# ishine/Prior-DiffuSE

Hardware: AMD Instinct MI355X
Metric: enhanced-audio sec/sec (RTF), 6-step fast sampling, B=32 (higher is better)
Workload: dtype f16x2; 1 GPU; B=32 x 4 s 16 kHz utterances per GPU, [B,2,401,161] spectrograms, GCRN prior + DiffUNet1 6-step sampling, STFT..ISTFT, seeded random weights; global_batch=32, frames=401, parallelism=batch-shard x1, graph=True, streams_per_gpu=1, batches_in_flight=3

## Files before the change

include/pdse.h:

```cpp
#ifndef PDSE_H
#define PDSE_H
#include <stdint.h>

#ifdef __cplusplus
extern "C" {
#endif

#define PDSE_ABI_VERSION 9

typedef void* pdse_stream_t;

enum pdse_act { PDSE_ACT_NONE = 0, PDSE_ACT_PRELU = 1, PDSE_ACT_ELU = 2, PDSE_ACT_SIGMOID = 3 };

enum pdse_epi {
  PDSE_EPI_LINEAR = 0,
  PDSE_EPI_GLU = 1,
  PDSE_EPI_BIGLU = 2
};

typedef struct pdse_src {
  const float* ptr;
  int64_t sb, sc, st, sf;
  int32_t C;
  int32_t act;
// ... 277 lines not shown
  int32_t split;
  const float* x;
  const float* wih;
  const float* bih;
} pdse_gru_desc;

typedef struct pdse_transpose_desc {
  const float* in;
  float* out;
  int32_t N, R, Cc, pad_;
} pdse_transpose_desc;

typedef struct pdse_crm_desc {
  const float* x;
  const float* o;
  const float* ri;
  float* out;
  float a1, b1, a2, b2, a3, b3;
  int32_t plane, B, mode, pad_;
} pdse_crm_desc;

typedef struct pdse_gcrnlast_desc {
  const float* in0;
  const float* in1;
  const float* w1;
  const float* w2;
  const float* fcT;
  const float* fcb;
  float* out;
  int64_t out_sb;
  float b1, b2, bn_scale, bn_shift;
  int32_t B, T;
  const float* fcp;
} pdse_gcrnlast_desc;

typedef struct pdse_tcm_desc {
  const float* x;
  const float* h;
  float* x_out;
  float* h_out;
  const float* wbr;
  const float* bmain;
  const float* bmask;
  const float* xf;
  const float* wc2;
  const float* bc2;
  const float* xf2;
  const float* wn1;
  const float* bn1;
  float slope_main, slope_mask, slope2;
  int32_t dil, B, T;
  const int32_t* frames;
} pdse_tcm_desc;

typedef struct pdse_tcm2_desc {
  const float* x;
  float* x_out;
  const uint16_t* hs;
  uint16_t* hs_out;
  const uint16_t* wbr;
  const uint16_t* wc2;
  const uint16_t* wn1;
  const float* par;
  float slope2, slope_main_next, slope_mask_next;
  int32_t dil, B, T, mode;
  int32_t np;
// ... 269 lines not shown
```

prior-diffuse_amd/_lib.py:

```python
import contextlib
import ctypes as C
import os

_HERE = os.path.dirname(os.path.abspath(__file__))
LIB_PATH = os.environ.get("PDSE_LIB") or os.path.join(_HERE, "libpdse.so")

ABI_VERSION = 9

ACT_NONE, ACT_PRELU, ACT_ELU, ACT_SIGMOID = 0, 1, 2, 3
EPI_LINEAR, EPI_GLU, EPI_BIGLU = 0, 1, 2
EW_DIV, EW_UPDATE, EW_UPDATE_FINAL, EW_COPY, EW_ADD_MUL = 0, 1, 2, 3, 4
(OP_GCONV, OP_TIME, OP_EW, OP_COMPAND, OP_WAVPREP, OP_OLA, OP_SIGMA, OP_LN, OP_LSTM,
 OP_ROWLN, OP_CHLN, OP_ATTN, OP_GRU, OP_GNCOMB, OP_AHAM, OP_QSAMPLE, OP_TRANSPOSE, OP_TCM, OP_CRM, OP_GCRNLAST,
 OP_MASKLOSS, OP_GLSTM, OP_TCM2, OP_BGLU, OP_PLANES, OP_GLSTMP, OP_TCM2S, OP_DENSE, OP_ROWLNB, OP_METRICS, OP_RESAMPLE, OP_RANGE) = range(32)
MASKLOSS_BLOCKS = 32

_fp = C.c_void_p
_i32, _i64, _f32 = C.c_int32, C.c_int64, C.c_float


class Src(C.Structure):
    _fields_ = [("ptr", _fp), ("sb", _i64), ("sc", _i64), ("st", _i64), ("sf", _i64),
                ("C", _i32), ("act", _i32), ("blk", _i32), ("pad_", _i32)]

# ... 164 lines not shown
class BgluDesc(C.Structure):
    _fields_ = [("hp", _fp), ("hp_sb", _i64), ("hp_Tp", _i32), ("hp_Fp", _i32), ("hp_t0", _i32), ("hp_f0", _i32),
                ("x0", Src), ("x1", Src), ("Tin", _i32), ("Fin", _i32), ("ntaps", _i32), ("sf_in", _i32),
                ("tap_dt", _i32 * 10), ("tap_df", _i32 * 10), ("p1mask", _i32), ("Fout1", _i32),
                ("B", _i32), ("Tout", _i32), ("Fout", _i32), ("np", _i32),
                ("w0", _fp), ("w1", _fp), ("w2", _fp), ("w3", _fp), ("wlc", _fp), ("wrc", _fp), ("wc2", _fp), ("wc2v", _fp),
                ("nx_w", _fp), ("bias0", _fp), ("bias1", _fp), ("bias0_t0", _fp), ("bias1_t0", _fp), ("bias_sb", _i64),
                ("blc", _fp), ("brc", _fp), ("bc2", _fp), ("slope", _f32), ("C2", _i32),
                ("out", _fp), ("out_sb", _i64), ("out_sc", _i64), ("out_st", _i64), ("out_sf", _i64), ("out_off", _i64),
                ("hp_par", _i32), ("nx_n", _i32),
                ("nx_hp", _fp), ("nx_hp_sb", _i64), ("nx_Tp", _i32), ("nx_Fp", _i32), ("nx_t0", _i32), ("nx_f0", _i32),
                ("nx_row0", _i32), ("nx_par", _i32),
                ("nx_add", _fp), ("add_sb", _i64), ("add_sc", _i64), ("add_st", _i64), ("add_sf", _i64),
                ("nx_out", _fp * 2), ("nx_sb", _i64 * 2), ("nx_sc", _i64 * 2), ("nx_st", _i64 * 2), ("nx_sf", _i64 * 2),
                ("nx_bias", _fp * 3), ("nx_bias_sb", _i64 * 3), ("skip_Fh", _i32), ("nx_items", _i32), ("qexp", _i32 * 4)]


class PlanesDesc(C.Structure):
    _fields_ = [("in_", _fp), ("in_sb", _i64), ("in_sc", _i64), ("in_st", _i64), ("in_sf", _i64),
                ("hp", _fp), ("hp_sb", _i64), ("hp_Tp", _i32), ("hp_Fp", _i32), ("hp_t0", _i32), ("hp_f0", _i32),
                ("B", _i32), ("T", _i32), ("F", _i32), ("np", _i32),
                ("in1", _fp), ("w", _fp * 2), ("bias", _fp * 2), ("bias_sb", _i64), ("hp1", _fp),
                ("cin0", _i32), ("cin1", _i32), ("nd", _i32), ("pad_", _i32)]


class CrmDesc(C.Structure):
    _fields_ = [("x", _fp), ("o", _fp), ("ri", _fp), ("out", _fp), ("a1", _f32), ("b1", _f32), ("a2", _f32), ("b2", _f32),
                ("a3", _f32), ("b3", _f32), ("plane", _i32), ("B", _i32), ("mode", _i32), ("pad_", _i32)]


class GcrnLastDesc(C.Structure):
    _fields_ = [("in0", _fp), ("in1", _fp), ("w1", _fp), ("w2", _fp), ("fcT", _fp), ("fcb", _fp), ("out", _fp),
                ("out_sb", _i64), ("b1", _f32), ("b2", _f32), ("bn_scale", _f32), ("bn_shift", _f32), ("B", _i32), ("T", _i32),
                ("fcp", _fp)]


class MetricsDesc(C.Structure):
    _fields_ = [("clean", _fp), ("proc", _fp), ("lens_host", _fp), ("lens", _fp), ("tables", _fp), ("frames", _fp),
                ("sorted", _fp), ("out", _fp), ("B", _i32), ("Lmax", _i32), ("Mmax", _i32), ("measures", _i32),
                ("stoi_tables", _fp), ("stoi_work", _fp), ("stoi_out", _fp)]


class ResampleDesc(C.Structure):
    _fields_ = [("pcm", _fp), ("offs", _fp), ("n_in_host", _fp), ("n_in", _fp), ("taps", _fp), ("out", _fp),
                ("pcm_bytes", _i64), ("B", _i32), ("Lmax", _i32), ("up", _i32), ("down", _i32), ("half", _i32),
                ("width", _i32), ("ch", _i32), ("pad_", _i32)]


class RangeRow(C.Structure):
    _fields_ = [("ptr", _fp), ("n", _i64), ("s0", _i64), ("s1", _i64), ("s2", _i64),
                ("n0", _i32), ("n1", _i32), ("n2", _i32), ("n3", _i32), ("i0", _i32), ("par_half", _i32),
                ("kind", _i32), ("exp", _i32), ("out_row", _i32), ("pad_", _i32)]


class RangeDesc(C.Structure):
    _fields_ = [("rows", _fp), ("out", _fp),
                ("nrows", _i32), ("out_rows", _i32), ("mode", _i32), ("blocks", _i32)]


RANGE_BINS = 32
RANGE_F32, RANGE_F16HI = 0, 1
RANGE_CLEAR, RANGE_ACCUMULATE = 0, 1
RANGE_NONFINITE = 2
RANGE_BINADE = (None, float("-inf")) + tuple(range(-14, 15)) + (15,)
RANGE_BIN_FULL = RANGE_BINADE.index(-2)
RANGE_BIN_TOP = RANGE_BINS - 1

# ... 209 lines not shown
```

prior-diffuse_amd/csrc/capi.hip:

```cpp
#include <hip/hip_runtime.h>
#include <stdint.h>
#include <stdio.h>
#include <string.h>

#include <new>
#include <string>
#include <vector>

#include "pdse.h"
#include "pdse_internal.h"

static thread_local std::string g_err;

void pdse_set_error(const char* msg) { g_err = msg ? msg : "unknown error"; }

int pdse_check_hip(hipError_t e, const char* what) {
  if (e == hipSuccess) return 0;
  g_err = std::string(what) + ": " + hipGetErrorString(e);
  return 1;
}

int pdse_check_launch(const char* what) { return pdse_check_hip(hipGetLastError(), what); }

int pdse_lds_attr(const void* fn, unsigned long long* mask, const char* what) {
// ... 54 lines not shown
};

static int op_size(int kind) {
  switch (kind) {
#define X(KIND, stem, entry) case PDSE_OP_##KIND: return (int)sizeof(pdse_##stem##_desc);
    PDSE_OPS(X)
#undef X
    default: return -1;
  }
}

static int launch_op(const pdse_op& op, hipStream_t s) {
  switch (op.kind) {
#define X(KIND, stem, entry) case PDSE_OP_##KIND: return pdse_##stem##_launch(&op.d.stem, s);
    PDSE_OPS(X)
#undef X
    default: pdse_set_error("plan: unknown op kind"); return 1;
  }
}

static bool names_odd_phase(const pdse_op& op) {
  return op.kind == PDSE_OP_GCONV && op.d.gconv.korder == 5 && op.d.gconv.p1mask != 0 && op.d.gconv.w2 == nullptr;
}

static int check_follows(const pdse_plan* p, const pdse_op& op) {
  if (p->ops.empty() || !names_odd_phase(p->ops.back())) return 0;
  if (op.kind != PDSE_OP_GCONV) {
    pdse_set_error("plan: the operator behind a gconv that names its odd phase (p1mask, korder 5) must be that phase");
    return 1;
  }
  return pdse_gconv_pair_check(&p->ops.back().d.gconv, &op.d.gconv);
}

static int launch_at(const pdse_plan* p, const int i, const int end, hipStream_t s, int* n) {
  const pdse_op& op = p->ops[i];
  *n = 1;
  if (names_odd_phase(op) && i + 1 < end) {
    *n = 2;
    return pdse_gconv4_pair_launch(&op.d.gconv, &p->ops[i + 1].d.gconv, s);
  }
  return launch_op(op, s);
}

template <typename D>
static int validate_desc(const D*) { return 0; }
static int validate_desc(const pdse_range_desc* d) { return pdse_range_validate(d); }

extern "C" {

int pdse_abi_version(void) { return PDSE_ABI_VERSION; }
const char* pdse_last_error(void) { return g_err.c_str(); }
int pdse_desc_size(int op_kind) { return op_size(op_kind); }

#define X(KIND, stem, entry) \
  int entry(const pdse_##stem##_desc* d, pdse_stream_t s) { return validate_desc(d) ? 1 : pdse_##stem##_launch(d, (hipStream_t)s); }
PDSE_OPS(X)
#undef X

int pdse_plan_create(pdse_plan** out) {
  if (!out) {
    pdse_set_error("plan_create: null out");
    return 1;
  }
  *out = new (std::nothrow) pdse_plan();
  if (!*out) {
    pdse_set_error("plan_create: out of memory");
    return 1;
  }
  return 0;
// ... 384 lines not shown
```

prior-diffuse_amd/csrc/gconv4.hip:

```cpp
#include <hip/hip_runtime.h>
#include <stdint.h>
#include <stdio.h>
#include <stdlib.h>

#include "pdse.h"
#include "pdse_internal.h"

#include "gconv_common.h"

#ifndef G4_CH
#define G4_CH 3
#endif

__device__ __forceinline__ void glds16_g4(const void* g, void* l) {
  __builtin_amdgcn_global_load_lds((const __attribute__((address_space(1))) void*)g, (__attribute__((address_space(3))) void*)l,
                                   16, 0, 0);
}

__device__ __forceinline__ float g4_load(const float* sbase, const unsigned byte_off) {
  float v;
  asm volatile("global_load_dword %0, %1, %2" : "=v"(v) : "v"(byte_off), "s"(sbase) : "memory");
  return v;
}
typedef float g4_f32x4 __attribute__((ext_vector_type(4)));
// ... 29 lines not shown
__device__ __forceinline__ void g4_lds_read3(const unsigned addr, u32x4 (&a)[3]) {
  asm volatile("ds_read_b128 %0, %3\n\tds_read_b128 %1, %3 offset:1024\n\tds_read_b128 %2, %3 offset:2048"
               : "=&v"(a[0]), "=&v"(a[1]), "=&v"(a[2])
               : "v"(addr)
               : "memory");
}
__device__ __forceinline__ void g4_lds_read3(const unsigned addr, u32x4 (&a)[2]) {
  asm volatile("ds_read_b128 %0, %2\n\tds_read_b128 %1, %2 offset:1024" : "=&v"(a[0]), "=&v"(a[1]) : "v"(addr) : "memory");
}
__device__ __forceinline__ void g4_lds_read3(const unsigned addr, u32x4 (&a)[1]) {
  asm volatile("ds_read_b128 %0, %1" : "=&v"(a[0]) : "v"(addr) : "memory");
}
template <int N, int NP>
__device__ __forceinline__ void g4_lds_wait(u32x4 (&a)[N][NP]) {
  asm volatile("s_waitcnt lgkmcnt(0)" ::: "memory");
#pragma unroll
  for (int i = 0; i < N; ++i)
#pragma unroll
    for (int p = 0; p < NP; ++p) asm volatile("" : "+v"(a[i][p]));
}
__device__ __forceinline__ f32x16 g4_mfma6(const u32x4 (&a)[3], const uint4 (&b)[3], f32x16 acc) {
  const uint4 a1 = make_uint4(a[0][0], a[0][1], a[0][2], a[0][3]), a2 = make_uint4(a[1][0], a[1][1], a[1][2], a[1][3]),
              a3 = make_uint4(a[2][0], a[2][1], a[2][2], a[2][3]);
  acc = mfma_bf16(a1, b[2], acc);
  acc = mfma_bf16(a3, b[0], acc);
  acc = mfma_bf16(a2, b[1], acc);
  acc = mfma_bf16(a1, b[1], acc);
  acc = mfma_bf16(a2, b[0], acc);
  acc = mfma_bf16(a1, b[0], acc);
  return acc;
}
__device__ __forceinline__ f32x16 g4_mfma6(const u32x4 (&a)[2], const uint4 (&b)[2], f32x16 acc) {
  const uint4 a1 = make_uint4(a[0][0], a[0][1], a[0][2], a[0][3]), a2 = make_uint4(a[1][0], a[1][1], a[1][2], a[1][3]);
  acc = mfma_f16(a2, b[0], acc);
  acc = mfma_f16(a1, b[1], acc);
  acc = mfma_f16(a1, b[0], acc);
  return acc;
}
__device__ __forceinline__ f32x16 g4_mfma6(const u32x4 (&a)[1], const uint4 (&b)[1], f32x16 acc) {
  return mfma_bf16(make_uint4(a[0][0], a[0][1], a[0][2], a[0][3]), b[0], acc);
}
__device__ __forceinline__ uint32_t g4_pack_bf16(const float a, const float b) {
  typedef float f32x2 __attribute__((ext_vector_type(2)));
  typedef __bf16 bf16x2 __attribute__((ext_vector_type(2)));
  const f32x2 v = {a, b};
  union { bf16x2 h; uint32_t u; } c;
  c.h = __builtin_convertvector(v, bf16x2);
  return c.u;
}
__device__ __forceinline__ void g4_split(const float (&x)[8], uint4 (&b)[3]) { split8(x, b[0], b[1], b[2]); }
__device__ __forceinline__ void g4_split(const float (&x)[8], uint4 (&b)[2]) { split8h(x, pow2i(PDSE_F16_ACT_EXP), b[0], b[1]); }
__device__ __forceinline__ void g4_split(const float (&x)[8], uint4 (&b)[1]) {
  b[0] = make_uint4(g4_pack_bf16(x[0], x[1]), g4_pack_bf16(x[2], x[3]), g4_pack_bf16(x[4], x[5]), g4_pack_bf16(x[6], x[7]));
}

struct g4_chunk {
  int s, tap, cb0, n, kb0;
};

__device__ long long* g_trace4 = nullptr;

template <int EPI, int MT, bool BLK, int NP = 3>
__global__ __launch_bounds__(512, 2) void gconv4_kernel(const pdse_gconv_desc d) {
  constexpr int FB = 64 * NP;
#ifdef PDSE_DIAG
  long long* const trace = g_trace4;
#else
  long long* const trace = nullptr;
#endif
  const long long c_start = trace ? clock64() : 0;
// ... 571 lines not shown
```

prior-diffuse_amd/csrc/gconv_common.h:

```cpp
#ifndef PDSE_GCONV_COMMON_H
#define PDSE_GCONV_COMMON_H
#include <hip/hip_runtime.h>
#include <type_traits>
#include <stdint.h>

#include "pdse.h"

typedef float f32x16 __attribute__((ext_vector_type(16)));
typedef float f32x4 __attribute__((ext_vector_type(4)));

__device__ __forceinline__ int rho(int r, int h) { return (r & 3) + 8 * (r >> 2) + 4 * h; }

__device__ __forceinline__ float fast_exp(float x) { return __builtin_amdgcn_exp2f(x * 1.44269504088896340736f); }
__device__ __forceinline__ float sigmoid_f(float x) { return __builtin_amdgcn_rcpf(1.0f + fast_exp(-x)); }

template <int ACT>
__device__ __forceinline__ float act_c(float y, float slope) {
  if constexpr (ACT == PDSE_ACT_PRELU) return y > 0.f ? y : slope * y;
  else if constexpr (ACT == PDSE_ACT_ELU) return y > 0.f ? y : fast_exp(y) - 1.0f;
  else if constexpr (ACT == PDSE_ACT_SIGMOID) return sigmoid_f(y);
  else return y;
}

__device__ const float pdse_zeros[32] __attribute__((aligned(16))) = {0.f, 0.f, 0.f, 0.f, 0.f, 0.f, 0.f, 0.f, 0.f, 0.f, 0.f, 0.f, 0.f, 0.f, 0.f, 0.f,
// ... 61 lines not shown
}

__device__ __forceinline__ void split8(const float (&x)[8], uint4& p1, uint4& p2, uint4& p3) {
#ifdef PDSE_ABLATE_SPLIT
  p1 = make_uint4(__float_as_uint(x[0]), __float_as_uint(x[1]), __float_as_uint(x[2]), __float_as_uint(x[3]));
  p2 = make_uint4(__float_as_uint(x[4]), __float_as_uint(x[5]), __float_as_uint(x[6]), __float_as_uint(x[7]));
  p3 = make_uint4(p1.x ^ p2.x, p1.y ^ p2.y, p1.z ^ p2.z, p1.w ^ p2.w);
  return;
#endif
  uint32_t q1[4], q2[4], q3[4];
#pragma unroll
  for (int i = 0; i < 4; ++i) {
    const float a = x[2 * i], b = x[2 * i + 1];
    const float ra = a - __uint_as_float(__float_as_uint(a) & 0xffff0000u);
    const float rb = b - __uint_as_float(__float_as_uint(b) & 0xffff0000u);
    const float sa = ra - __uint_as_float(__float_as_uint(ra) & 0xffff0000u);
    const float sb = rb - __uint_as_float(__float_as_uint(rb) & 0xffff0000u);
    q1[i] = __builtin_amdgcn_perm(__float_as_uint(b), __float_as_uint(a), 0x07060302u);
    q2[i] = __builtin_amdgcn_perm(__float_as_uint(rb), __float_as_uint(ra), 0x07060302u);
    q3[i] = __builtin_amdgcn_perm(__float_as_uint(sb), __float_as_uint(sa), 0x07060302u);
  }
  p1 = make_uint4(q1[0], q1[1], q1[2], q1[3]);
  p2 = make_uint4(q2[0], q2[1], q2[2], q2[3]);
  p3 = make_uint4(q3[0], q3[1], q3[2], q3[3]);
}

typedef _Float16 f16x8 __attribute__((ext_vector_type(8)));

__device__ __forceinline__ f32x16 mfma_f16(const uint4& a, const uint4& b, const f32x16 c) {
  union { uint4 u; f16x8 v; } A, B;
  A.u = a;
  B.u = b;
  return __builtin_amdgcn_mfma_f32_32x32x16_f16(A.v, B.v, c, 0, 0, 0);
}

__device__ __forceinline__ float pow2i(const int e) { return __uint_as_float((uint32_t)(127 + e) << 23); }


__device__ __forceinline__ void split8h(const float (&x)[8], const float sc, uint4& p1, uint4& p2) {
  typedef float f32x2 __attribute__((ext_vector_type(2)));
  typedef _Float16 f16x2 __attribute__((ext_vector_type(2)));
  uint32_t q1[4], q2[4];
#pragma unroll
  for (int i = 0; i < 4; ++i) {
    const f32x2 t = {x[2 * i] * sc, x[2 * i + 1] * sc};
    union { f16x2 h; uint32_t u; } hi, lo;
    hi.h = __builtin_convertvector(t, f16x2);
    const f32x2 r = t - __builtin_convertvector(hi.h, f32x2);
    lo.h = __builtin_convertvector(r, f16x2);
    q1[i] = hi.u;
    q2[i] = lo.u;
  }
  p1 = make_uint4(q1[0], q1[1], q1[2], q1[3]);
  p2 = make_uint4(q2[0], q2[1], q2[2], q2[3]);
}

__device__ __forceinline__ f32x16 mfma6(const uint4* w, const uint4& b1, const uint4& b2, const uint4& b3, f32x16 acc) {
  const uint4 a1 = w[0], a2 = w[64], a3 = w[128];
  acc = mfma_bf16(a1, b3, acc);
  acc = mfma_bf16(a3, b1, acc);
  acc = mfma_bf16(a2, b2, acc);
  acc = mfma_bf16(a1, b2, acc);
  acc = mfma_bf16(a2, b1, acc);
  acc = mfma_bf16(a1, b1, acc);
  return acc;
}
// ... 545 lines not shown
```

prior-diffuse_amd/csrc/misc.hip:

```cpp
#include <hip/hip_runtime.h>
#include <stdint.h>

#include "pdse.h"
#include "pdse_internal.h"

#define REQ(cond, msg)          \
  do {                          \
    if (!(cond)) {              \
      pdse_set_error(msg);      \
      return 1;                 \
    }                           \
  } while (0)

__device__ __forceinline__ float silu_f(float x) { return x * (1.0f / (1.0f + expf(-x))); }

__global__ __launch_bounds__(1024) void time_embed_kernel(const pdse_time_desc d) {
  __shared__ float x0[128];
  __shared__ float y1[512];
  __shared__ float y2[512];
  const int b = blockIdx.x, j = threadIdx.x;
  const float t = d.t[b];
  if (j < 128) {
    float fl = floorf(t), ce = ceilf(t);
    int lo = (int)fl, hi = (int)ce;
    lo = min(max(lo, 0), d.max_steps - 1);
    hi = min(max(hi, 0), d.max_steps - 1);
    const float low = d.table[lo * 128 + j], high = d.table[hi * 128 + j];
    x0[j] = low + (high - low) * (t - fl);
  }
  __syncthreads();
  if (j < 512) {
    float s = d.b1[j];
    for (int i = 0; i < 128; ++i) s += d.p1T[i * 512 + j] * x0[i];
    y1[j] = silu_f(s);
  }
  __syncthreads();
  if (j < 512) {
// ... 313 lines not shown
    float t1, t2;
    if (d.mode == 0) {
      const float diff = d.label[off + i] - d.init[off + i];
      t1 = a * diff;
      t2 = s * d.noise[off + i];
    } else if (d.mode == 1) {
      t1 = a * d.label[off + i];
      const float ni = d.noise[off + i] + d.init[off + i];
      t2 = s * ni;
    } else {
      t1 = a * d.label[off + i];
      t2 = s * d.noise[off + i];
    }
    d.out[off + i] = t1 + t2;
  }
}

int pdse_qsample_launch(const pdse_qsample_desc* d, hipStream_t s) {
  REQ(d && d->label && d->noise && d->a && d->s && d->out, "qsample: null pointer");
  REQ(d->mode >= 0 && d->mode <= 2 && (d->mode == 2 || d->init), "qsample: mode 0 / 1 need init");
  REQ(d->B > 0 && d->B <= 65535 && d->plane > 0, "qsample: bad sizes");
  int bx = (int)((d->plane + 255) / 256);
  if (bx > 128) bx = 128;
  hipLaunchKernelGGL(qsample_kernel, dim3(bx, d->B), dim3(256), 0, s, *d);
  return pdse_check_launch("qsample");
}

#define GL_F 161
#define GL_FI 80
#define GL_KQ 21
#define GL_YB 132
__device__ __forceinline__ float gl_exp(float x) { return __builtin_amdgcn_exp2f(x * 1.44269504088896340736f); }

__global__ __launch_bounds__(512, 4) void gcrnlast_kernel(const pdse_gcrnlast_desc d) {
  typedef float f32x16 __attribute__((ext_vector_type(16)));
  __shared__ __attribute__((aligned(16))) float xs[2][2][32 * GL_FI];
  __shared__ __attribute__((aligned(16))) float ys[GL_KQ * 2 * GL_YB];
  __shared__ __attribute__((aligned(16))) float4 wl4[2][32];
  const int tid = threadIdx.x, lane = tid & 63, wave = tid >> 6;
  const int o = tid & 255, rr = tid >> 8;
  const bool act = o < GL_F;
  const bool odd = (o & 1) != 0;
  if (tid < 64) {
    const int c = tid & 31, par = tid >> 5;
    wl4[par][c] = par ? make_float4(d.w1[3 * c + 1], 0.f, d.w2[3 * c + 1], 0.f) : make_float4(d.w1[3 * c], d.w1[3 * c + 2], d.w2[3 * c], d.w2[3 * c + 2]);
  }
  for (int e = tid; e < GL_KQ * 2 * GL_YB; e += 512) ys[e] = 0.f;
  const int64_t plane = (int64_t)d.T * GL_FI;
  const int rows = d.B * d.T, ntiles = (rows + 31) >> 5;
  auto fetch = [&](const int row, float (&v)[10]) {
    const int rw = row < rows ? row : 0;
    const int b = rw / d.T, t = rw - b * d.T;
#pragma unroll
    for (int i = 0; i < 10; ++i) {
      const int e = o + 256 * i;
      const int c = e / GL_FI, f = e - c * GL_FI;
      v[i] = c < 16 ? d.in0[((int64_t)b * 16 + c) * plane + (int64_t)t * GL_FI + f]
                    : d.in1[((int64_t)b * 16 + (c - 16)) * plane + (int64_t)t * GL_FI + f];
    }
  };
  for (int tile = blockIdx.x; tile < ntiles; tile += gridDim.x) {
    const int row0 = tile * 32;
    float nxt[10];
    fetch(row0 + rr, nxt);
    __syncthreads();
    for (int it = 0; it < 16; ++it) {
      float* const xb = xs[it & 1][rr];
#pragma unroll
      for (int i = 0; i < 10; ++i) {
        const int e = o + 256 * i;
        const float v = nxt[i];
        xb[e] = e < 16 * GL_FI ? v : (v > 0.f ? v : gl_exp(v) - 1.0f);
      }
      if (it + 1 < 16) fetch(row0 + 2 * (it + 1) + rr, nxt);
      __syncthreads();
      if (act) {
        const int j = o >> 1;
        const bool has0 = odd || j < GL_FI, has2 = !odd && j >= 1;
        const int j0 = has0 ? j : GL_FI - 1, j2 = has2 ? j - 1 : 0;
        float m = 0.f, g = 0.f;
#pragma unroll 8
        for (int k = 0; k < 32; ++k) {
          const float4 w = wl4[odd ? 1 : 0][k];
          const float x0 = has0 ? xb[k * GL_FI + j0] : 0.f, x2 = has2 ? xb[k * GL_FI + j2] : 0.f;
          m += x0 * w.x + x2 * w.y;
          g += x0 * w.z + x2 * w.w;
        }
        float y = (m + d.b1) * __builtin_amdgcn_rcpf(1.0f + gl_exp(-(g + d.b2)));
        y = y * d.bn_scale + d.bn_shift;
        y = y > 0.f ? y : gl_exp(y) - 1.0f;
        ys[(2 * (o >> 3) + (o & 1)) * GL_YB + (2 * it + rr) * 4 + ((o >> 1) & 3)] = y;
      }
    }
    __syncthreads();
    if (wave < 6) {
      f32x16 acc;
#pragma unroll
      for (int r = 0; r < 16; ++r) acc[r] = 0.f;
      const float4* const B4 = reinterpret_cast<const float4*>(d.fcp) + (size_t)wave * GL_KQ * 64 + lane;
      const float* const A1 = ys + (lane >> 5) * GL_YB + (lane & 31) * 4;
#pragma unroll 7
      for (int kq = 0; kq < GL_KQ; ++kq) {
        const float4 bv = B4[(size_t)kq * 64];
        const float4 av = *reinterpret_cast<const float4*>(A1 + kq * 2 * GL_YB);
        acc = __builtin_amdgcn_mfma_f32_32x32x2f32(av.x, bv.x, acc, 0, 0, 0);
        acc = __builtin_amdgcn_mfma_f32_32x32x2f32(av.y, bv.y, acc, 0, 0, 0);
        acc = __builtin_amdgcn_mfma_f32_32x32x2f32(av.z, bv.z, acc, 0, 0, 0);
        acc = __builtin_amdgcn_mfma_f32_32x32x2f32(av.w, bv.w, acc, 0, 0, 0);
      }
      const int ob = 32 * wave + (lane & 31);
      if (ob < GL_F) {
        const float bias = d.fcb[ob];
#pragma unroll
        for (int r = 0; r < 16; ++r) {
          const int row = row0 + (r & 3) + 8 * (r >> 2) + 4 * (lane >> 5);
          if (row < rows) {
            const int b = row / d.T, t = row - b * d.T;
            d.out[(int64_t)b * d.out_sb + (int64_t)t * GL_F + ob] = acc[r] + bias;
          }
        }
      }
    }
  }
}

int pdse_gcrnlast_launch(const pdse_gcrnlast_desc* d, hipStream_t s) {
  REQ(d && d->in0 && d->in1 && d->w1 && d->w2 && d->fcT && d->fcp && d->fcb && d->out, "gcrn_last: null pointer");
  REQ(d->B > 0 && d->T > 0 && (int64_t)d->B * d->T < (1ll << 31), "gcrn_last: bad sizes");
  const int ntiles = (d->B * d->T + 31) / 32;
  hipLaunchKernelGGL(gcrnlast_kernel, dim3(ntiles < 512 ? ntiles : 512), dim3(512), 0, s, *d);
  return pdse_check_launch("gcrn_last");
}

__device__ __forceinline__ double block_sum_256(double v, double* lds) {
  for (int o = 32; o > 0; o >>= 1) v += __shfl_down(v, o);
  const int lane = threadIdx.x & 63, wave = threadIdx.x >> 6;
  if (lane == 0) lds[wave] = v;
  __syncthreads();
  double r = 0.0;
  if (threadIdx.x == 0) r = ((lds[0] + lds[1]) + lds[2]) + lds[3];
  return r;
}

__global__ __launch_bounds__(256) void maskloss_partial_kernel(const pdse_maskloss_desc d) {
  __shared__ double lds[4];
  const int b = blockIdx.y;
  const int fr = min(max(d.frames[b], 0), d.T);
  const int64_t plane = (int64_t)d.T * d.F, live = (int64_t)fr * d.F;
  double acc = 0.0;
  for (int c = 0; c < d.C; ++c) {
    const int64_t base = ((int64_t)b * d.C + c) * plane;
    for (int64_t i = (int64_t)blockIdx.x * 256 + threadIdx.x; i < live; i += (int64_t)gridDim.x * 256) {
      const float e = d.esti[base + i] - d.label[base + i];
      acc += (double)e * (double)e;
    }
  }
  const double tot = block_sum_256(acc, lds);
  if (threadIdx.x == 0) d.partial[(int64_t)b * gridDim.x + blockIdx.x] = tot;
}

__global__ __launch_bounds__(256) void maskloss_final_kernel(const pdse_maskloss_desc d) {
  __shared__ double lds[4];
  const int n = d.B * PDSE_MASKLOSS_BLOCKS;
// ... 18 lines not shown
```

prior-diffuse_amd/nets.py:

```python
import ctypes as C

import numpy as np
import torch

from . import _lib as L
from . import packing as P

F0 = 161
BIG = 1 << 30

TAG_NONE, TAG_EPS_BLOCK, TAG_EPS_CONV1, TAG_TCM, TAG_PRIOR, TAG_LSTM, TAG_SIGNAL, TAG_EW = range(8)


class WeightBank:

    def __init__(self):
        self.items = {}
        self.keep = []
        self.owners = []

    def token(self, obj):
        if obj is None:
            return None
        for i, o in enumerate(self.owners):
# ... 92 lines not shown
        self.descs.append((desc, tag))
        if self.plan is not None:
            self.plan.add(desc, tag)
        for op in self.f16x2_operands(desc):
            self._audit_ops.setdefault((op[0], op[1]), op)

    def named(self, name, t):
        self._audit_names[t.data_ptr()] = (name, t)
        return t

    @staticmethod
    def f16x2_operands(desc):
        out = []
        if isinstance(desc, L.BgluDesc) and desc.np == 2:
            if desc.hp:
                F_ = desc.hp_Fp - 2 * desc.hp_f0
                box = P.hp_box(desc.B, desc.hp_Tp - desc.hp_t0, F_, 2, par=bool(desc.hp_par))
                out.append((desc.hp + 2 * box["off"], L.RANGE_F16HI, box, ""))
            else:
                out += [(desc.x0.ptr, L.RANGE_F32, None, ""), (desc.x1.ptr, L.RANGE_F32, None, "")]
        elif isinstance(desc, L.Tcm2Desc) and desc.np == 2:
            out.append((desc.x, L.RANGE_F32, None, ""))
            if desc.mode == 0:
                for br, suffix in enumerate((".main", ".mask")):
                    box = P.tcm2_hs_box(desc.B, desc.T, 2, br)
                    out.append((desc.hs + 2 * box["off"], L.RANGE_F16HI, box, suffix))
        elif isinstance(desc, L.Tcm2sDesc):
            for i in range(desc.n):
                out += PlanBase.f16x2_operands(desc.blk[i])
        elif isinstance(desc, L.GconvDesc) and desc.korder == 5:
            out += [(s_.ptr, L.RANGE_F32, None, "") for s_ in (desc.in0, desc.in1) if s_.ptr]
        elif isinstance(desc, L.DenseDesc) and desc.np == 2:
            out.append((desc.D, L.RANGE_F32, None, ""))
        return [o for o in out if o[0]]

    def audited(self):
        out, seen = [], set()
        for addr, kind, box, suffix in self._audit_ops.values():
            hit = next(((n, t) for n, t in self._audit_names.values()
                        if t.data_ptr() <= addr < t.data_ptr() + t.numel() * t.element_size()), None)
            if hit is None:
                raise RuntimeError("range audit: the f16x2 operand at 0x%x lies in no buffer the builder named (PlanBase.named)" % addr)
            name, t = hit
            key = (name + suffix, kind)
            if key in seen:
                continue
            seen.add(key)
            out.append((name + suffix, t, kind, P.F16_ACT_EXP if kind == L.RANGE_F32 else 0,
                        None if box is None else dict(box, off=(addr - t.data_ptr()) // 2)))
        return out

    def finish(self):
        if self.plan is not None:
            self.plan.keep(self.ctx.keep, self.ctx.bank)

    def src(self, t, C_, sb, sc, st, sf, off=0, act=L.ACT_NONE, blk=0):
        return L.Src(Ctx.ptr(t, off), sb, sc, st, sf, C_, act, blk, 0)

    def gconv(self, *, in0, in1=None, Tin, Fin, taps, sf_in, W, Cout, bias0=None, bias0_sb=0,
              bias1=None, bias1_sb=0, epi=L.EPI_LINEAR, act=L.ACT_NONE, act_slope=0.0,
              padrow=None, padrow_sb=0, padrow_off=0, cin1=False, resid=None, out,
              out_strides, out_off=0, out_cr=1, B, Tout, Fout, tag=TAG_NONE, bias0_off=0, phase1=None, nx=None,
              bias1_off=0, bias_t0=None, label="gconv", s3=False, s3g=False, has_xf=False, flat=False):
        ctx = self.ctx
        d = L.GconvDesc()
        d.in0 = in0
# ... 695 lines not shown
                p = "%s.de%d.0" % (de, k)
                if k > 1:
                    o, ooff = self.dec[n & 1], 0
                    fn = lambda Fo: nchw_out(64, T, Fo)
                    bn, pr = "%s.de%d.2" % (de, k), "%s.de%d.3.weight" % (de, k)
                else:
                    o, ooff = out, di * T * F0
                    fn = lambda Fo: nchw_out(2, T, Fo)
                    bn, pr = None, None
                nx = None
                if chained and k > 1:
                    Fo = 2 * (Fin - 1) + 3
                    wn = lambda de=de, k=k: self.w("%s.de%d.0.conv1.weight" % (de, k - 1))[:, :, 0, 0].T[:, :64]
                    nx = dict(keep=False, row0=-1, tiles=[dict(wfn=wn, bias=self.zero32, out=Hn, add=self.Pskip[di][k - 1],
                                                                strides=(32 * T * Fo, T * Fo, Fo, 2))])
                Fin = self._biconvtransglu(step, 5 + 5 * di + n, p, k, in0, in1, Fin, o, fn, bn, pr, out_off=ooff, H=Hc,
                                           do_conv1=(k == 5 or not chained), nx=nx)
                if chained:
                    Hc, Hn = Hn, Hc
                in0 = self.src(o, 64, *nchw(64, T, Fin))
        return out


class GcrnPlan(PlanBase):
    fused_last = True
    fused_glstm = True
    split_bf16 = True
    gemm_planes = 2
    block8 = True
    fuse_phases = True
    flat_proj = True
    persist_lstm = True
    chunk_proj = True
    CHUNK_TC = 32
    PERSIST_MAX_B = 4
    ENC_C = [2, 16, 32, 64, 128, 256]
    ENC_F = [161, 80, 39, 19, 9, 4]

    def __init__(self, ctx, sd, B, T, plan=None, split_bf16=None, exclusive=False, planes=None):
        if split_bf16 is not None:
            self.split_bf16 = bool(split_bf16)
        if planes is not None:
            if planes not in (1, 2, 3) or (planes in (1, 2) and not self.split_bf16):
                raise ValueError("planes is 3 (bf16x3), 2 (f16x2) or 1 (bf16 mode); the one- and two-plane forms run on the GEMM kernels (split_bf16)")
            self.gemm_planes = int(planes)
        self.persist = bool(self.persist_lstm and self.fused_glstm and exclusive and B <= self.PERSIST_MAX_B and not self.force_generic)
        self.exclusive = bool(exclusive)
        self.chunk = bool(self.chunk_proj and self.fused_glstm and not exclusive and not self.persist and not self.force_generic
                          and T >= 2 * self.CHUNK_TC)
        super().__init__(ctx, plan, ns=(ctx.bank.token(sd), self.fused_last, self.fused_glstm, self.split_bf16, self.block8, self.persist,
                                        self.gemm_planes))
        self.sd, self.B, self.T = sd, B, T
        a = ctx.alloc
        self.Bp = Bp = (B + 31) // 32 * 32
        self.status = None
        self.x = a(B, 2, T, F0)
        self.out = a(B, 2, T, F0)
        self.e = [a(B, self.ENC_C[i + 1], T, self.ENC_F[i + 1]) for i in range(5)]
        self.gx = a(2, T, 2048, Bp, zero=True)
        R = 2 * self.CHUNK_TC if self.chunk else 2
        self.hT = a(R, 2, 512, Bp, zero=True)
        self.cst = a(2, 512, Bp, zero=True)
        self.y = a(B, T, 1024)
        if self.persist:
            bq = 1 << (B - 1).bit_length()
            self.gran = torch.zeros(4 * 1024 * bq, dtype=torch.int64, device=ctx.device)
            self.status = torch.zeros(4, dtype=torch.int32, device=ctx.device)
            ctx.keep += [self.gran, self.status]
        elif self.fused_glstm and not self.force_generic:
            self.hT2, self.cst2 = a(2, 2, 512, Bp, zero=True), a(2, 512, Bp, zero=True)
            self.gx2, self.part = a(R, 2, 2048, Bp, zero=True), a(R, 2, 64, Bp, 2, zero=True)
        else:
            self.yn = a(B, 1024, T)
        self.glstm = a(B, 256, T, 4)
        self.d = [a(B, 128, T, 9), a(B, 64, T, 19), a(B, 32, T, 39), a(B, 16, T, 80), a(B, 1, T, 161)]
        for i, t_ in enumerate(self.e):
            self.named("gcrn.e%d" % (i + 1), t_)
        self.named("gcrn.glstm", self.glstm)
        for i, t_ in enumerate(self.d[:4]):
            self.named("gcrn.d%d" % (5 - i), t_)
        self.named("gcrn.x", self.x)

# ... 109 lines not shown
            s = self.src(self.e[4], 128, *e_lay[4][0], off=128 * g * T * 4, blk=8 if blk else 0)
            return s, T, 4, [(0, f) for f in range(4)], wk, T, 1, 2048 * Bp, 0

        if self.persist:
            self._glstm_persistent(proj1)
        elif self.fused_glstm and not self.force_generic:
            self._glstm_wavefront(proj1)
        else:
            self._lstm_layer("lstm_list1", proj1, y_su=2, y_sg=1)
            self._ln("glstm.ln1", self.yn, 1024 * T, T, 0, 1, 1)

            def proj2(g):
                s = self.src(self.yn, 512, 1024 * T, T, 0, 1, off=512 * g * T)
                return s, 1, T, [(0, 0)], (lambda Wih: Wih.T), 1, T, 0, 2048 * Bp

            self._lstm_layer("lstm_list2", proj2, y_su=1, y_sg=512)
        if blk:
            self._ln("glstm.ln2", self.glstm, 256 * T * 4, T * 4 * 8, 8, 4 * 8, 4, blk=8)
        else:
            self._ln("glstm.ln2", self.glstm, 256 * T * 4, T * 4, 1, 4, 4)

        dec = [(5, 512, 128), (4, 256, 64), (3, 128, 32), (2, 64, 16), (1, 32, 1)]
        for br in (1, 2):
            in0 = self.src(self.glstm, 256, *(nc8(256, T, 4) if blk else nchw(256, T, 4)), blk=8 if blk else 0)
            in1 = self.src(self.e[4], 256, *e_lay[4][0], blk=8 if blk else 0)
            Fin = 4
            for n, (k, ci, co) in enumerate(dec):
                p = "conv%d_t_%d" % (k, br)
                Fout = 2 * (Fin - 1) + 3 + (1 if k == 2 else 0)
                if k == 1 and self.fused_last and not self.force_generic:
                    g = L.GcrnLastDesc()
                    self.apply(g, self.fields(p + ".last", lambda p=p, br=br: P.gcrn_last_fields(self.sd, p, br)))
                    g.in0, g.in1 = self.d[3].data_ptr(), self.e[0].data_ptr()
                    g.out, g.out_sb = Ctx.ptr(out, (br - 1) * T * F0), 2 * T * F0
                    g.B, g.T = B, T
                    self.add(g, TAG_PRIOR)
                    break
                dblk = blk and k >= 3
                fuse = self.fuse_phases and self.split_bf16 and self.gemm_planes == 2 and not self.force_generic
                ist, (osb, osc, olo, ost, osf), ocr = lay(dblk, co, Fout)
                for phase in (0, 1):
                    kk, taps = P.convT_phase_taps(1, 3, phase)
                    self.gconv(in0=in0, in1=in1, Tin=T, Fin=Fin, taps=taps, sf_in=1, Cout=co, epi=L.EPI_GLU, act=L.ACT_ELU,
                               W=lambda p=p, k=k, br=br, kk=kk: dict(
                                   wk0=P.convT_kmat(self.sd[p + ".conv1.weight"], kk),
                                   wk1=P.convT_kmat(self.sd[p + ".conv2.weight"], kk), bias0=self.w(p + ".conv1.bias"),
                                   bias1=self.w(p + ".conv2.bias"), post=P.bn_fold(self.sd, "bn%d_t_%d" % (k, br))),
                               out=self.d[n], out_strides=(osb, osc, olo, ost, 2 * osf), out_off=phase * osf, out_cr=ocr, B=B,
                               Tout=T, Fout=(Fout - phase + 1) // 2, tag=TAG_PRIOR, label="%s.ph%d" % (p, phase),
                               s3g=self.split_bf16, phase1=dict(mask=1, Fout1=Fout // 2) if phase == 0 and fuse and co <= 32 else None)
                Fin = Fout
                if k > 1:
                    in0 = self.src(self.d[n], co, *ist, blk=8 if dblk else 0)
                    skip = self.e[k - 2]
                    sblk = e_lay[k - 2][2] == 8
                    in1 = self.src(skip, co, *e_lay[k - 2][0], act=L.ACT_ELU, blk=8 if sblk else 0)
            else:
                self.gconv(in0=self.src(self.d[4], 1, *nchw(1, T, F0)), Tin=T, Fin=F0, taps=[(0, f) for f in range(F0)],
                           sf_in=1, W=lambda br=br: dict(wk0=self.w("fc%d.weight" % br).T, bias0=self.w("fc%d.bias" % br)),
                           Cout=F0, cin1=True, out=out, out_strides=(2 * T * F0, 1, 0, F0, 0), out_off=(br - 1) * T * F0, B=B,
                           Tout=T, Fout=1, tag=TAG_PRIOR, label="fc%d" % br)
        return out


class StftPlan(PlanBase):

    def __init__(self, ctx, B, L_, plan=None, normalize=True, split_bf16=False, reflect_own=False):
        super().__init__(ctx, plan, ns=("stft", bool(split_bf16)))
        self.split_bf16 = bool(split_bf16)
        if L_ <= 160:
            raise ValueError(f"utterance of {L_} samples: the centred STFT reflects 160 samples on each side (torch.stft "
                             "raises for the same input)")
        self.B, self.L = B, L_
        self.T = 1 + L_ // 160
        self.wav = ctx.alloc(B, L_)
        self.xpad = ctx.alloc(B, L_ + 320)
        self.c = ctx.alloc(B)
        self.lens = torch.full((B,), L_, dtype=torch.int32, device=ctx.device)
        ctx.keep.append(self.lens)
        self.feat = ctx.alloc(B, 2, self.T, F0)
        self.normalize = normalize
        self.reflect_own = bool(reflect_own)

# ... 424 lines not shown
```

Before: 10090 audio_s/s.

## Fuse last 16-channel transposed-conv stage into the GCRN final kernel

Adds a tail mode to the gcrn_last kernel that computes the preceding 16-channel transposed-conv GLU stage (both phases) per row tile with MFMA and writes its output straight into shared memory, instead of round-tripping through the d[3] buffer. The launcher detects the gconv pair followed by a matching gcrn_last op and launches only the fused kernel, skipping two gconv phase launches. This removes a global write/read of the intermediate activation and two launches. In exchange the fused kernel does more work per tile, uses only 5 waves for the tail compute, and adds barriers, which may hurt occupancy or overlap.

```diff
diff --git a/include/pdse.h b/include/pdse.h
--- a/include/pdse.h
+++ b/include/pdse.h
@@ -333,6 +333,19 @@
   float b1, b2, bn_scale, bn_shift;
   int32_t B, T;
   const float* fcp;
+  const float* t_in0;
+  const float* t_in1;
+  const float* t_w0e;
+  const float* t_w1e;
+  const float* t_w0o;
+  const float* t_w1o;
+  const float* t_bias0;
+  const float* t_bias1;
+  const float* t_post_scale;
+  const float* t_post_shift;
+  int64_t t_sb0, t_sc0, t_st0, t_sf0;
+  int64_t t_sb1, t_sc1, t_st1, t_sf1;
+  int32_t tail, t_wexp_e, t_wexp_o, pad_;
 } pdse_gcrnlast_desc;
 
 typedef struct pdse_tcm_desc {
diff --git a/prior-diffuse_amd/_lib.py b/prior-diffuse_amd/_lib.py
--- a/prior-diffuse_amd/_lib.py
+++ b/prior-diffuse_amd/_lib.py
@@ -220,7 +220,12 @@
 class GcrnLastDesc(C.Structure):
     _fields_ = [("in0", _fp), ("in1", _fp), ("w1", _fp), ("w2", _fp), ("fcT", _fp), ("fcb", _fp), ("out", _fp),
                 ("out_sb", _i64), ("b1", _f32), ("b2", _f32), ("bn_scale", _f32), ("bn_shift", _f32), ("B", _i32), ("T", _i32),
-                ("fcp", _fp)]
+                ("fcp", _fp),
+                ("t_in0", _fp), ("t_in1", _fp), ("t_w0e", _fp), ("t_w1e", _fp), ("t_w0o", _fp), ("t_w1o", _fp),
+                ("t_bias0", _fp), ("t_bias1", _fp), ("t_post_scale", _fp), ("t_post_shift", _fp),
+                ("t_sb0", _i64), ("t_sc0", _i64), ("t_st0", _i64), ("t_sf0", _i64),
+                ("t_sb1", _i64), ("t_sc1", _i64), ("t_st1", _i64), ("t_sf1", _i64),
+                ("tail", _i32), ("t_wexp_e", _i32), ("t_wexp_o", _i32), ("pad_", _i32)]
 
 
 class MetricsDesc(C.Structure):
diff --git a/prior-diffuse_amd/csrc/capi.hip b/prior-diffuse_amd/csrc/capi.hip
--- a/prior-diffuse_amd/csrc/capi.hip
+++ b/prior-diffuse_amd/csrc/capi.hip
@@ -110,9 +110,22 @@
   return pdse_gconv_pair_check(&p->ops.back().d.gconv, &op.d.gconv);
 }
 
+static bool absorbs_pair(const pdse_op& last, const pdse_op& d, const pdse_op& e) {
+  if (last.kind != PDSE_OP_GCRNLAST || e.kind != PDSE_OP_GCONV) return false;
+  const pdse_gcrnlast_desc& g = last.d.gcrnlast;
+  const pdse_gconv_desc &a = d.d.gconv, &b = e.d.gconv;
+  return g.tail == 1 && g.t_in0 == a.in0.ptr && g.t_in1 == a.in1.ptr && g.t_w0e == a.w0 && g.t_w1e == a.w1 && g.t_w0o == b.w0 &&
+         g.t_w1o == b.w1 && g.t_wexp_e == a.wexp && g.t_wexp_o == b.wexp && g.in0 == a.out && a.out == b.out && a.B == g.B &&
+         a.Tout == g.T;
+}
+
 static int launch_at(const pdse_plan* p, const int i, const int end, hipStream_t s, int* n) {
   const pdse_op& op = p->ops[i];
   *n = 1;
+  if (names_odd_phase(op) && i + 2 < end && absorbs_pair(p->ops[i + 2], op, p->ops[i + 1])) {
+    *n = 3;
+    return launch_op(p->ops[i + 2], s);
+  }
   if (names_odd_phase(op) && i + 1 < end) {
     *n = 2;
     return pdse_gconv4_pair_launch(&op.d.gconv, &p->ops[i + 1].d.gconv, s);
diff --git a/prior-diffuse_amd/csrc/gconv4.hip b/prior-diffuse_amd/csrc/gconv4.hip
--- a/prior-diffuse_amd/csrc/gconv4.hip
+++ b/prior-diffuse_amd/csrc/gconv4.hip
@@ -85,10 +85,7 @@
 }
 __device__ __forceinline__ f32x16 g4_mfma6(const u32x4 (&a)[2], const uint4 (&b)[2], f32x16 acc) {
   const uint4 a1 = make_uint4(a[0][0], a[0][1], a[0][2], a[0][3]), a2 = make_uint4(a[1][0], a[1][1], a[1][2], a[1][3]);
-  acc = mfma_f16(a2, b[0], acc);
-  acc = mfma_f16(a1, b[1], acc);
-  acc = mfma_f16(a1, b[0], acc);
-  return acc;
+  return mfma3_f16(a1, a2, b[0], b[1], acc);
 }
 __device__ __forceinline__ f32x16 g4_mfma6(const u32x4 (&a)[1], const uint4 (&b)[1], f32x16 acc) {
   return mfma_bf16(make_uint4(a[0][0], a[0][1], a[0][2], a[0][3]), b[0], acc);
diff --git a/prior-diffuse_amd/csrc/gconv_common.h b/prior-diffuse_amd/csrc/gconv_common.h
--- a/prior-diffuse_amd/csrc/gconv_common.h
+++ b/prior-diffuse_amd/csrc/gconv_common.h
@@ -117,6 +117,13 @@
   A.u = a;
   B.u = b;
   return __builtin_amdgcn_mfma_f32_32x32x16_f16(A.v, B.v, c, 0, 0, 0);
+}
+
+__device__ __forceinline__ f32x16 mfma3_f16(const uint4& a1, const uint4& a2, const uint4& b1, const uint4& b2, f32x16 acc) {
+  acc = mfma_f16(a2, b1, acc);
+  acc = mfma_f16(a1, b2, acc);
+  acc = mfma_f16(a1, b1, acc);
+  return acc;
 }
 
 __device__ __forceinline__ float pow2i(const int e) { return __uint_as_float((uint32_t)(127 + e) << 23); }
diff --git a/prior-diffuse_amd/csrc/misc.hip b/prior-diffuse_amd/csrc/misc.hip
--- a/prior-diffuse_amd/csrc/misc.hip
+++ b/prior-diffuse_amd/csrc/misc.hip
@@ -3,6 +3,8 @@
 
 #include "pdse.h"
 #include "pdse_internal.h"
+
+#include "gconv_common.h"
 
 #define REQ(cond, msg)          \
   do {                          \
@@ -382,8 +384,8 @@
 #define GL_YB 132
 __device__ __forceinline__ float gl_exp(float x) { return __builtin_amdgcn_exp2f(x * 1.44269504088896340736f); }
 
+template <bool TAIL>
 __global__ __launch_bounds__(512, 4) void gcrnlast_kernel(const pdse_gcrnlast_desc d) {
-  typedef float f32x16 __attribute__((ext_vector_type(16)));
   __shared__ __attribute__((aligned(16))) float xs[2][2][32 * GL_FI];
   __shared__ __attribute__((aligned(16))) float ys[GL_KQ * 2 * GL_YB];
   __shared__ __attribute__((aligned(16))) float4 wl4[2][32];
@@ -402,11 +404,78 @@
     const int rw = row < rows ? row : 0;
     const int b = rw / d.T, t = rw - b * d.T;
 #pragma unroll
-    for (int i = 0; i < 10; ++i) {
+    for (int i = TAIL ? 5 : 0; i < 10; ++i) {
       const int e = o + 256 * i;
       const int c = e / GL_FI, f = e - c * GL_FI;
       v[i] = c < 16 ? d.in0[((int64_t)b * 16 + c) * plane + (int64_t)t * GL_FI + f]
                     : d.in1[((int64_t)b * 16 + (c - 16)) * plane + (int64_t)t * GL_FI + f];
+    }
+  };
+  auto tail_rows = [&](const int first) {
+    const int n = 32 * wave + (lane & 31), hh = lane >> 5;
+    const int rl = n / 40, j = n - 40 * rl;
+    f32x16 ae, ao;
+    if (wave < 5) {
+      const int row = first + rl, rw = row < rows ? row : 0;
+      const int b = rw / d.T, t = rw - b * d.T;
+#pragma unroll
+      for (int r = 0; r < 16; ++r) ae[r] = ao[r] = 0.f;
+      const bool gate = (lane & 16) != 0;
+      const int wl = lane - (gate ? 16 : 0);
+      const uint4* const we = reinterpret_cast<const uint4*>(gate ? d.t_w1e : d.t_w0e) + wl;
+      const uint4* const wo = reinterpret_cast<const uint4*>(gate ? d.t_w1o : d.t_w0o) + wl;
+#pragma unroll 1
+      for (int s = 0; s < 2; ++s) {
+        const float* const sp = (s ? d.t_in1 : d.t_in0) + (int64_t)b * (s ? d.t_sb1 : d.t_sb0) + (int64_t)t * (s ? d.t_st1 : d.t_st0);
+        const int ssc = (int)(s ? d.t_sc1 : d.t_sc0), ssf = (int)(s ? d.t_sf1 : d.t_sf0);
+#pragma unroll
+        for (int tap = 0; tap < 2; ++tap) {
+          const int fin = j - tap;
+          const bool inb = fin >= 0 && fin < 39;
+#pragma unroll
+          for (int cb = 0; cb < 2; ++cb) {
+            const float* const q = sp + ((inb ? fin : 0) * ssf + (2 * cb + hh) * ssc);
+            const float4 v0 = *reinterpret_cast<const float4*>(q), v1 = *reinterpret_cast<const float4*>(q + 4);
+            float x[8] = {v0.x, v0.y, v0.z, v0.w, v1.x, v1.y, v1.z, v1.w};
+#pragma unroll
+            for (int e = 0; e < 8; ++e) x[e] = inb ? x[e] : 0.f;
+            if (s) {
+#pragma unroll
+              for (int e = 0; e < 8; ++e) x[e] = x[e] < 0.f ? fast_exp(x[e]) - 1.0f : x[e];
+            }
+            uint4 b1, b2;
+            split8h(x, pow2i(PDSE_F16_ACT_EXP), b1, b2);
+            const uint4* const fe = we + (size_t)((s * 2 + tap) * 2 + cb) * 128;
+            ae = mfma3_f16(fe[0], fe[64], b1, b2, ae);
+            if (tap == 0) {
+              const uint4* const fo = wo + (size_t)(s * 2 + cb) * 128;
+              ao = mfma3_f16(fo[0], fo[64], b1, b2, ao);
+            }
+          }
+        }
+      }
+      const float ue = pow2i(-(PDSE_F16_ACT_EXP + d.t_wexp_e)), uo = pow2i(-(PDSE_F16_ACT_EXP + d.t_wexp_o));
+#pragma unroll
+      for (int r = 0; r < 16; ++r) {
+        ae[r] *= ue;
+        ao[r] *= uo;
+      }
+    }
+    __syncthreads();
+    if (wave < 5) {
+      float* const xo = xs[rl >> 1][rl & 1] + 2 * j;
+      const float *pb0 = d.t_bias0 + 4 * hh, *pb1 = d.t_bias1 + 4 * hh, *ps = d.t_post_scale + 4 * hh, *pt = d.t_post_shift + 4 * hh;
+#pragma unroll
+      for (int r = 0; r < 8; ++r) {
+        float y = ae[r] + pb0[PDSE_KR(r)];
+        y = y * sigmoid_f(ae[r + 8] + pb1[PDSE_KR(r)]);
+        y = y * ps[PDSE_KR(r)] + pt[PDSE_KR(r)];
+        xo[(PDSE_KR(r) + 4 * hh) * GL_FI] = act_c<PDSE_ACT_ELU>(y, 0.f);
+        float z = ao[r] + pb0[PDSE_KR(r)];
+        z = z * sigmoid_f(ao[r + 8] + pb1[PDSE_KR(r)]);
+        z = z * ps[PDSE_KR(r)] + pt[PDSE_KR(r)];
+        xo[(PDSE_KR(r) + 4 * hh) * GL_FI + 1] = act_c<PDSE_ACT_ELU>(z, 0.f);
+      }
     }
   };
   for (int tile = blockIdx.x; tile < ntiles; tile += gridDim.x) {
@@ -415,9 +484,10 @@
     fetch(row0 + rr, nxt);
     __syncthreads();
     for (int it = 0; it < 16; ++it) {
+      if (TAIL && !(it & 1)) tail_rows(row0 + 2 * it);
       float* const xb = xs[it & 1][rr];
 #pragma unroll
-      for (int i = 0; i < 10; ++i) {
+      for (int i = TAIL ? 5 : 0; i < 10; ++i) {
         const int e = o + 256 * i;
         const float v = nxt[i];
         xb[e] = e < 16 * GL_FI ? v : (v > 0.f ? v : gl_exp(v) - 1.0f);
@@ -475,10 +545,25 @@
 }
 
 int pdse_gcrnlast_launch(const pdse_gcrnlast_desc* d, hipStream_t s) {
-  REQ(d && d->in0 && d->in1 && d->w1 && d->w2 && d->fcT && d->fcp && d->fcb && d->out, "gcrn_last: null pointer");
+  REQ(d && d->in1 && d->w1 && d->w2 && d->fcT && d->fcp && d->fcb && d->out, "gcrn_last: null pointer");
   REQ(d->B > 0 && d->T > 0 && (int64_t)d->B * d->T < (1ll << 31), "gcrn_last: bad sizes");
+  REQ(d->tail == 0 || d->tail == 1, "gcrn_last: tail is 0 or 1");
   const int ntiles = (d->B * d->T + 31) / 32;
-  hipLaunchKernelGGL(gcrnlast_kernel, dim3(ntiles < 512 ? ntiles : 512), dim3(512), 0, s, *d);
+  const dim3 grid(ntiles < 512 ? ntiles : 512);
+  if (d->tail) {
+    REQ(d->t_in0 && d->t_in1 && d->t_w0e && d->t_w1e && d->t_w0o && d->t_w1o && d->t_bias0 && d->t_bias1 && d->t_post_scale &&
+            d->t_post_shift,
+        "gcrn_last: tail = 1 needs the sources, packed weights, biases and folded BatchNorm of the 16-channel stage");
+    REQ(!((d->t_sb0 | d->t_sc0 | d->t_st0 | d->t_sf0 | d->t_sb1 | d->t_sc1 | d->t_st1 | d->t_sf1) & 3) &&
+            !((reinterpret_cast<uintptr_t>(d->t_in0) | reinterpret_cast<uintptr_t>(d->t_in1) | reinterpret_cast<uintptr_t>(d->t_w0e) |
+               reinterpret_cast<uintptr_t>(d->t_w1e) | reinterpret_cast<uintptr_t>(d->t_w0o) | reinterpret_cast<uintptr_t>(d->t_w1o)) & 15),
+        "gcrn_last: the tail's sources are channel-blocked (strides in multiples of 4 floats), sources and weights 16-byte aligned");
+    REQ(d->t_wexp_e >= -40 && d->t_wexp_e <= 40 && d->t_wexp_o >= -40 && d->t_wexp_o <= 40, "gcrn_last: tail weight exponent out of range");
+    hipLaunchKernelGGL(gcrnlast_kernel<true>, grid, dim3(512), 0, s, *d);
+    return pdse_check_launch("gcrn_last tail");
+  }
+  REQ(d->in0, "gcrn_last: null pointer");
+  hipLaunchKernelGGL(gcrnlast_kernel<false>, grid, dim3(512), 0, s, *d);
   return pdse_check_launch("gcrn_last");
 }
 
diff --git a/prior-diffuse_amd/nets.py b/prior-diffuse_amd/nets.py
--- a/prior-diffuse_amd/nets.py
+++ b/prior-diffuse_amd/nets.py
@@ -148,6 +148,8 @@
             out += [(s_.ptr, L.RANGE_F32, None, "") for s_ in (desc.in0, desc.in1) if s_.ptr]
         elif isinstance(desc, L.DenseDesc) and desc.np == 2:
             out.append((desc.D, L.RANGE_F32, None, ""))
+        elif isinstance(desc, L.GcrnLastDesc) and desc.tail:
+            out += [(desc.t_in0, L.RANGE_F32, None, ""), (desc.t_in1, L.RANGE_F32, None, "")]
         return [o for o in out if o[0]]
 
     def audited(self):
@@ -909,6 +911,8 @@
     flat_proj = True
     persist_lstm = True
     chunk_proj = True
+    fused_tail = True
+    TAIL_MIN_ROWS = 1024
     CHUNK_TC = 32
     PERSIST_MAX_B = 4
     ENC_C = [2, 16, 32, 64, 128, 256]
@@ -925,6 +929,8 @@
         self.exclusive = bool(exclusive)
         self.chunk = bool(self.chunk_proj and self.fused_glstm and not exclusive and not self.persist and not self.force_generic
                           and T >= 2 * self.CHUNK_TC)
+        self.tail = bool(self.fused_tail and B * T >= self.TAIL_MIN_ROWS and self.split_bf16 and self.gemm_planes == 2
+                         and self.fused_last and self.block8 and not self.force_generic)
         super().__init__(ctx, plan, ns=(ctx.bank.token(sd), self.fused_last, self.fused_glstm, self.split_bf16, self.block8, self.persist,
                                         self.gemm_planes))
         self.sd, self.B, self.T = sd, B, T
@@ -1100,6 +1106,14 @@
                     g = L.GcrnLastDesc()
                     self.apply(g, self.fields(p + ".last", lambda p=p, br=br: P.gcrn_last_fields(self.sd, p, br)))
                     g.in0, g.in1 = self.d[3].data_ptr(), self.e[0].data_ptr()
+                    if self.tail:
+                        pe, po = tail_ph
+                        g.tail, g.t_in0, g.t_in1 = 1, pe.in0.ptr, pe.in1.ptr
+                        g.t_sb0, g.t_sc0, g.t_st0, g.t_sf0 = pe.in0.sb, pe.in0.sc, pe.in0.st, pe.in0.sf
+                        g.t_sb1, g.t_sc1, g.t_st1, g.t_sf1 = pe.in1.sb, pe.in1.sc, pe.in1.st, pe.in1.sf
+                        g.t_w0e, g.t_w1e, g.t_w0o, g.t_w1o = pe.w0, pe.w1, po.w0, po.w1
+                        g.t_bias0, g.t_bias1, g.t_post_scale, g.t_post_shift = pe.bias0, pe.bias1, pe.post_scale, pe.post_shift
+                        g.t_wexp_e, g.t_wexp_o = pe.wexp, po.wexp
                     g.out, g.out_sb = Ctx.ptr(out, (br - 1) * T * F0), 2 * T * F0
                     g.B, g.T = B, T
                     self.add(g, TAG_PRIOR)
@@ -1107,16 +1121,19 @@
                 dblk = blk and k >= 3
                 fuse = self.fuse_phases and self.split_bf16 and self.gemm_planes == 2 and not self.force_generic
                 ist, (osb, osc, olo, ost, osf), ocr = lay(dblk, co, Fout)
+                tail_ph = []
                 for phase in (0, 1):
                     kk, taps = P.convT_phase_taps(1, 3, phase)
-                    self.gconv(in0=in0, in1=in1, Tin=T, Fin=Fin, taps=taps, sf_in=1, Cout=co, epi=L.EPI_GLU, act=L.ACT_ELU,
-                               W=lambda p=p, k=k, br=br, kk=kk: dict(
-                                   wk0=P.convT_kmat(self.sd[p + ".conv1.weight"], kk),
-                                   wk1=P.convT_kmat(self.sd[p + ".conv2.weight"], kk), bias0=self.w(p + ".conv1.bias"),
-                                   bias1=self.w(p + ".conv2.bias"), post=P.bn_fold(self.sd, "bn%d_t_%d" % (k, br))),
-                               out=self.d[n], out_strides=(osb, osc, olo, ost, 2 * osf), out_off=phase * osf, out_cr=ocr, B=B,
-                               Tout=T, Fout=(Fout - phase + 1) // 2, tag=TAG_PRIOR, label="%s.ph%d" % (p, phase),
-                               s3g=self.split_bf16, phase1=dict(mask=1, Fout1=Fout // 2) if phase == 0 and fuse and co <= 32 else None)
+                    tail_ph.append(self.gconv(
+                        in0=in0, in1=in1, Tin=T, Fin=Fin, taps=taps, sf_in=1, Cout=co,
+                        epi=L.EPI_GLU, act=L.ACT_ELU,
+                        W=lambda p=p, k=k, br=br, kk=kk: dict(
+                            wk0=P.convT_kmat(self.sd[p + ".conv1.weight"], kk),
+                            wk1=P.convT_kmat(self.sd[p + ".conv2.weight"], kk), bias0=self.w(p + ".conv1.bias"),
+                            bias1=self.w(p + ".conv2.bias"), post=P.bn_fold(self.sd, "bn%d_t_%d" % (k, br))),
+                        out=self.d[n], out_strides=(osb, osc, olo, ost, 2 * osf), out_off=phase * osf, out_cr=ocr, B=B,
+                        Tout=T, Fout=(Fout - phase + 1) // 2, tag=TAG_PRIOR, label="%s.ph%d" % (p, phase),
+                        s3g=self.split_bf16, phase1=dict(mask=1, Fout1=Fout // 2) if phase == 0 and fuse and co <= 32 else None))
                 Fin = Fout
                 if k > 1:
                     in0 = self.src(self.d[n], co, *ist, blk=8 if dblk else 0)
```

Result: no change. 10110 audio_s/s (median of 6 runs) (+0.3%).
